# evandez/neuron-descriptions

Measured on AMD Instinct MI355X. Metric: neuron-descriptions/sec (whole node), 4096 neurons x k=15 exemplars, higher is better.
Workload: dtype f32-equivalent: operands split into (hi,lo) f16 pairs (22 significant bits), 3 f16 MFMAs per product, f32 accumulate

## Files before the change

### include/milan_hip.h

```cpp
#ifndef MILAN_HIP_H
#define MILAN_HIP_H

#include <stddef.h>
#include <stdint.h>

#ifdef __cplusplus
extern "C" {
#endif

#if defined(__GNUC__)
#pragma GCC visibility push(default)
#endif

#define MILAN_ABI_VERSION 11

enum {
  MILAN_OK = 0,
  MILAN_ERR_ARG = -1,
  MILAN_ERR_SHAPE = -2,
  MILAN_ERR_STATE = -3,
  MILAN_ERR_WORKSPACE = -4,
  MILAN_ERR_NO_LM = -5
};

// ... 164 lines not shown
                                 milan_stream stream);

size_t milan_exemplar_sort_workspace(int n_units, int64_t n, int pairs);
int milan_exemplar_sketch_compact(const float* src, int64_t src_capacity,
                                  int64_t n, int n_units, int offset, float* dst,
                                  int64_t dst_capacity, int64_t position,
                                  float* extremes, void* workspace,
                                  size_t workspace_bytes, milan_stream stream);

size_t milan_exemplar_sketch_add_workspace(int n_units, int64_t supplied,
                                           const int64_t* capacities,
                                           int n_levels);
int milan_exemplar_sketch_add(const float* hiddens, int batch, int channels, int hw,
                              const int32_t* units, int n_units, int64_t first,
                              int64_t* consumed, float* const* levels,
                              int64_t* firstfree, const int64_t* capacities,
                              int n_levels, const uint8_t* randbits,
                              int64_t n_randbits, int64_t* currentbit,
                              float* extremes, void* workspace,
                              size_t workspace_bytes, milan_stream stream);

int milan_exemplar_rows_extremes(const float* rows, int64_t n_rows, int n_units,
                                 float* extremes, milan_stream stream);

enum { MILAN_SKETCH_COMPACT = 0, MILAN_SKETCH_INSERT = 1, MILAN_SKETCH_MOVE = 2,
       MILAN_SKETCH_HALVE = 3 };
typedef struct milan_sketch_op {
  int32_t kind, src, dst, offset, extremes, reserved;
  int64_t n, position, capacity;
} milan_sketch_op;
int milan_exemplar_sketch_plan_shift(int64_t resolution, int64_t buffersize,
                                     int full_rate, int n_levels,
                                     const int64_t* capacities,
                                     const int64_t* firstfree,
                                     int (*draw_bit)(void*), void* user,
                                     milan_sketch_op* ops, int max_ops, int* n_ops,
                                     int64_t* capacities_out, int64_t* firstfree_out,
                                     int* n_levels_out);

int milan_exemplar_sketch_quantile(const float* const* levels,
                                   const int64_t* firstfree,
                                   const int64_t* capacities, int n_levels,
                                   int n_units, float* extremes, float q,
                                   float* out, void* workspace,
                                   size_t workspace_bytes, milan_stream stream);

int milan_exemplar_render(const float* hiddens, int batch, int channels, int h,
                          int w, const float* images, int img_h, int img_w,
                          const int32_t* cells, int n_cells, const float* levels,
                          const float* mul3, const float* add3, int out_size,
                          int k, uint8_t* out_images, uint8_t* out_masks,
                          uint8_t* out_masked, milan_stream stream);

int milan_conv2d_nhwc(const float* x, int n, int h, int w, int cin,
                      const float* weight_oihw, const float* bias, int cout,
                      int kh, int kw, int stride, int pad, int relu,
                      const float* residual, float* y, int precision,
                      milan_stream stream);

size_t milan_lm_train_workspace_bytes(const milan_ctx* ctx, int rows, int L);
int milan_lm_nll(milan_ctx* ctx, const float* const* params, int n_params,
                 const int64_t* inputs, const int64_t* targets, int rows, int L,
                 float* loss_sum_and_count, void* workspace,
                 size_t workspace_bytes, milan_stream stream);
int milan_lm_train_step(milan_ctx* ctx, const float* const* params,
                        float* const* grads, int n_params,
                        const int64_t* inputs, const int64_t* targets, int rows,
                        int L, float dropout, uint64_t seed,
                        float* loss_sum_and_count, void* workspace,
                        size_t workspace_bytes, milan_stream stream);

size_t milan_lm_grad_workspace_bytes(const milan_ctx* ctx, int rows, int L);
int milan_lm_forward_train(milan_ctx* ctx, const float* const* params,
                           int n_params, const int64_t* inputs, int rows, int L,
                           float dropout, uint64_t seed, float* logprobs_out,
                           float* picked_out, const int64_t* targets,
                           void* workspace, size_t workspace_bytes,
                           milan_stream stream);
int milan_lm_backward(milan_ctx* ctx, const float* const* params,
                      float* const* grads, int n_params, const int64_t* inputs,
                      int rows, int L, float dropout, uint64_t seed,
                      const float* dlogprobs, const float* dpicked,
                      const int64_t* targets, void* workspace,
                      size_t workspace_bytes, milan_stream stream);

size_t milan_decoder_train_workspace_bytes(const milan_ctx* ctx, int rows,
                                           int k, int L);
int milan_decoder_nll(milan_ctx* ctx, const float* const* params, int n_params,
                      const float* features, const int64_t* targets, int rows,
                      int k, int L, float* loss_terms, void* workspace,
                      size_t workspace_bytes, milan_stream stream);
int milan_decoder_train_step(milan_ctx* ctx, const float* const* params,
                             float* const* grads, int n_params,
                             const float* features, const int64_t* targets,
                             int rows, int k, int L, float dropout,
                             uint64_t seed, float regularization_weight,
                             float* loss_terms, void* workspace,
                             size_t workspace_bytes, milan_stream stream);

size_t milan_decoder_grad_workspace_bytes(const milan_ctx* ctx, int rows, int k,
                                          int L);
int milan_decoder_forward_train(milan_ctx* ctx, const float* const* params,
                                int n_params, const float* features,
                                const int64_t* targets, int rows, int k, int L,
                                float dropout, uint64_t seed,
                                float* logprobs_out, float* attentions_out,
// ... 96 lines not shown
```

### neuron-descriptions_amd/csrc/api.hip

```cpp
#include "common.h"

#include <cstdarg>
#include <cstdio>
#include <cstring>

namespace milan {

static thread_local char g_err[1024] = "";

void set_error(const char* fmt, ...) {
  va_list ap;
  va_start(ap, fmt);
  vsnprintf(g_err, sizeof(g_err), fmt, ap);
  va_end(ap);
}

int dev_alloc(milan_ctx* c, void** p, size_t bytes) {
  if (bytes == 0) bytes = 16;
  MILAN_CHECK_HIP(hipMalloc(p, (bytes + 255) & ~size_t(255)));
  c->owned.push_back(*p);
  return 0;
}

__global__ void absmax_kernel(const float* __restrict__ w, long n,
// ... 313 lines not shown
                 int length, int beam_size, int mi, float temperature,
                 int group_size, int64_t* tokens, float* scores,
                 float* predictions, float* attentions, int64_t* beam_tokens,
                 float* beam_scores, int32_t* out_len, void* workspace,
                 size_t workspace_bytes, milan_stream stream) {
  MILAN_REQUIRE(c && features, MILAN_ERR_ARG, "milan_decode: null argument");
  set_status_word(c->status);
  Arena a;
  MILAN_TRY(make_arena(workspace, workspace_bytes, &a));
  DecodeCall d{features, n, k, strategy, length, beam_size, mi, temperature,
               group_size, tokens, scores, predictions, attentions, beam_tokens,
               beam_scores, out_len, workspace, workspace_bytes,
               (hipStream_t)stream, c->precision};
  return decode_maybe_graph(c, d);
}

int milan_set_graph_capture(milan_ctx* c, int enable) {
  MILAN_REQUIRE(c, MILAN_ERR_ARG, "null ctx");
  c->graph_capture = enable != 0;
  if (!enable) {
    for (auto& g : c->graphs)
      if (g.exec) (void)hipGraphExecDestroy(g.exec);
    c->graphs.clear();
  }
  return 0;
}

int milan_graph_stats(const milan_ctx* c, long long* captures, long long* replays) {
  MILAN_REQUIRE(c, MILAN_ERR_ARG, "null ctx");
  if (captures) *captures = c->graph_captures;
  if (replays) *replays = c->graph_replays;
  return 0;
}

int milan_lm_score(milan_ctx* c, const int64_t* seqs, int rows, int L,
                   const int32_t* seq_len, float* out, void* workspace,
                   size_t workspace_bytes, milan_stream stream) {
  MILAN_REQUIRE(c && seqs && out, MILAN_ERR_ARG, "milan_lm_score: null argument");
  set_status_word(c->status);
  Arena a;
  MILAN_TRY(make_arena(workspace, workspace_bytes, &a));
  return decoder_lm_score(c, seqs, rows, L, seq_len, out, a, (hipStream_t)stream);
}

int milan_lm_logprobs(milan_ctx* c, const int64_t* seqs, int rows, int L,
                      float* out, void* workspace, size_t workspace_bytes,
                      milan_stream stream) {
  MILAN_REQUIRE(c && seqs && out, MILAN_ERR_ARG,
                "milan_lm_logprobs: null argument");
  set_status_word(c->status);
  Arena a;
  MILAN_TRY(make_arena(workspace, workspace_bytes, &a));
  return decoder_lm_logprobs(c, seqs, rows, L, out, a, (hipStream_t)stream);
}

int milan_conv2d_nhwc(const float* x, int n, int h, int w, int cin,
                      const float* weight_oihw, const float* bias, int cout,
                      int kh, int kw, int stride, int pad, int relu,
                      const float* residual, float* y, int precision,
                      milan_stream stream) {
  MILAN_REQUIRE(x && weight_oihw && y, MILAN_ERR_ARG, "conv2d: null argument");
  set_status_word(nullptr);
  const bool force_strip = precision == 3, tap_major = precision == 4;
  if (force_strip || tap_major) precision = MILAN_PRECISION_SPLIT_F16;
  MILAN_REQUIRE(!force_strip || MILAN_EXPERIMENTS, MILAN_ERR_ARG,
                "conv2d: the LDS-strip 3x3 kernel is only in an experiments build "
                "(make EXPERIMENTS=1)");
  MILAN_REQUIRE(precision == MILAN_PRECISION_F32 || cin % 32 == 0,
                MILAN_ERR_SHAPE, "conv2d: split-f16 needs cin %% 32 == 0");
  MILAN_REQUIRE(cin % 4 == 0 && n > 0 && cout > 0, MILAN_ERR_SHAPE,
                "conv2d: cin must be a multiple of 4");
  hipStream_t s = (hipStream_t)stream;
  const int K = kh * kw * cin, Kp = (K + 31) / 32 * 32;
  float *wp = nullptr, *zero = nullptr, *xs = nullptr, *wsp = nullptr, *ws3 = nullptr, *wst = nullptr;
  MILAN_CHECK_HIP(hipMalloc((void**)&wp, sizeof(float) * (size_t)cout * Kp));
  MILAN_CHECK_HIP(hipMalloc((void**)&zero, 256));
  MILAN_CHECK_HIP(hipMemsetAsync(zero, 0, 256, s));
  int r = pack_conv_plain(weight_oihw, cout, cin, kh, kw, wp, s);
  if (r == 0) {
    GemmArgs g{};
    const int ho = (h + 2 * pad - kh) / stride + 1, wo = (w + 2 * pad - kw) / stride + 1;
    g.A = x; g.W = wp; g.bias = bias; g.aux = residual; g.C = y;
    g.M = n * ho * wo; g.N = cout; g.K = K; g.Kp = Kp; g.ldc = cout; g.ldaux = cout;
    g.H = h; g.Wd = w; g.Cin = cin; g.Ho = ho; g.Wo = wo; g.KH = kh; g.KW = kw;
    g.stride = stride; g.pad = pad; g.a_pix_stride = cin;
    g.a_img_stride = (long)h * w * cin;
    g.epilogue = residual ? EPI_BIAS_RES_RELU : (relu ? EPI_BIAS_RELU : EPI_BIAS);
    g.zero = zero;
    if (precision == MILAN_PRECISION_SPLIT_F16) {
      const long rows = (long)n * h * w;
      hipError_t e1 = hipMalloc((void**)&xs, sizeof(float) * (size_t)rows * cin);
      hipError_t e2 = hipMalloc((void**)&wsp, sizeof(float) * (size_t)cout * Kp);
      if (e1 != hipSuccess || e2 != hipSuccess) {
        set_error("conv2d: out of memory");
        r = (int)hipErrorOutOfMemory;
      } else {
        r = launch_f32_to_split(x, cin, xs, cin, rows, cin, 1.f, s);
        if (r == 0)
          r = split_weight_into(wp, cout, Kp, wsp, &g.acc_scale,
                                reinterpret_cast<unsigned int*>(zero) + 32, s);
        g.A = xs; g.W = wsp; g.a_split = 1;
        if (r == 0 && !tap_major && kh * kw > 1 && kh * kw <= 32 && K == Kp) {
          if (hipMalloc((void**)&wst, sizeof(float) * (size_t)cout * Kp) == hipSuccess) {
            r = make_slice_major(wsp, cout, kh * kw, cin, 4, 2, wst, s);
            g.Wt = wst;
          }
// ... 155 lines not shown
```

### neuron-descriptions_amd/csrc/common.h

```cpp
#pragma once
#include <hip/hip_runtime.h>
#include <stdint.h>
#include <stddef.h>
#include <string>
#include <vector>
#include <map>

#include "../../include/milan_hip.h"

#ifndef MILAN_EXPERIMENTS
#define MILAN_EXPERIMENTS 0
#endif

namespace milan {

void set_error(const char* fmt, ...);
#define MILAN_CHECK_HIP(expr)                                              \
  do {                                                                     \
    hipError_t _e = (expr);                                                \
    if (_e != hipSuccess) {                                                \
      milan::set_error("%s:%d: %s -> %s", __FILE__, __LINE__, #expr,       \
                       hipGetErrorString(_e));                             \
      return (int)_e;                                                      \
    }                                                                      \
// ... 353 lines not shown
  float *bn1_scale = nullptr, *bn1_shift = nullptr;
  float act_scale = 32.f;
  int act_scale_log2 = 5;
  float *bn1_scale_s = nullptr, *bn1_shift_s = nullptr;
  unsigned* stem_lut = nullptr;
  unsigned* status = nullptr;
  unsigned* calib = nullptr;
  std::vector<milan::Bottleneck> blocks[4];
  float mean[3] = {0.485f, 0.456f, 0.406f}, stdv[3] = {0.229f, 0.224f, 0.225f};
  milan::LinearW init_h, init_c, q2h, k2h, gate, lstm_ih, lstm_hh, out;
  milan::LinearW lstm_cat;
  float *att_w = nullptr, *att_b = nullptr;
  float* embedding = nullptr;
  std::vector<milan::LinearW> lm_ih, lm_hh;
  std::vector<milan::LinearW> lm_cat;
  milan::LinearW lm_out;
  float* lm_embedding = nullptr;
};

namespace milan {
int dev_alloc(milan_ctx* c, void** p, size_t bytes);
int make_split_weight(milan_ctx* c, const float* w, int n, int kp, float** ws,
                      float* ws_inv, hipStream_t s);
int pack_conv_plain(const float* w_oihw, int cout, int cin, int kh, int kw,
                    float* wp, hipStream_t s);
int encoder_finalize(milan_ctx* c, hipStream_t s);
int encoder_rescale(milan_ctx* c, hipStream_t s);
int make_slice_major(const float* ws, int cout, int taps, int cin, int gps, int gb, float* dst,
                     hipStream_t s);
int make_chunk_major(const float* ws, int cout, int cin, float* dst,
                     hipStream_t s);
size_t encoder_workspace(const milan_ctx* c, int n_images, int H, int W);
int encoder_run_spatial(milan_ctx* c, const void* images, int image_dtype,
                        const void* masks, int mask_dtype, int n, int H, int W,
                        float* out, milan::Arena& ws, hipStream_t s);
int encoder_run(milan_ctx* c, const void* images, int image_dtype,
                const void* masks, int mask_dtype, int n_images, int H, int W,
                float* features, Arena& ws, hipStream_t s);
int decoder_finalize(milan_ctx* c, hipStream_t s);
size_t decoder_workspace(const milan_ctx* c, int n, int k, int beam, int length);
int decoder_init_state(milan_ctx* c, const float* features, int n, int k,
                       float* h, float* cc, Arena& ws, hipStream_t s);
int decoder_step(milan_ctx* c, const float* features, int rows, int k,
                 const int64_t* tokens, const float* h, const float* cc,
                 float* h_lm, float* c_lm, float temperature,
                 float* predictions, float* attentions, float* h_out,
                 float* c_out, Arena& ws, hipStream_t s);
int decoder_decode(milan_ctx* c, const float* features, int n, int k,
                   int strategy, int length, int beam, int mi,
                   float temperature, int group_size, int64_t* tokens,
                   float* scores, float* predictions, float* attentions,
                   int64_t* beam_tokens, float* beam_scores, int32_t* out_len,
                   Arena& ws, hipStream_t s);
int decoder_lm_logprobs(milan_ctx* c, const int64_t* seqs, int rows, int L,
                        float* out, milan::Arena& ws, hipStream_t s);
int decoder_lm_score(milan_ctx* c, const int64_t* seqs, int rows, int L,
                     const int32_t* seq_len, float* out, Arena& ws,
                     hipStream_t s);
}
```

### neuron-descriptions_amd/csrc/decoder.hip

```cpp
#include "common.h"
#include <limits>
#include <optional>

namespace milan {

static constexpr float kFloatMin = -3.402823466e+38f;

static const Tensor* find(milan_ctx* c, const std::string& name) {
  auto it = c->raw.find(name);
  return it == c->raw.end() ? nullptr : &it->second;
}

__global__ void pack_rows_kernel(const float* __restrict__ src, int n, int k,
                                 int kp, float* __restrict__ dst) {
  const long total = (long)n * kp;
  for (long idx = blockIdx.x * (long)blockDim.x + threadIdx.x; idx < total;
       idx += (long)gridDim.x * blockDim.x) {
    const int r = idx / kp, col = idx - (long)r * kp;
    dst[idx] = col < k ? src[(long)r * k + col] : 0.f;
  }
}

__device__ inline int lstm_source_row(int i, int hidden) {
  if (!hidden) return i;
// ... 569 lines not shown
  if (lm_logits) {
    const float* y = lm_logits + (long)r * V;
    float my = -INFINITY;
    for (int i = tid; i < V; i += 256) my = fmaxf(my, y[i]);
    my = block_max(my, red);
    float sy = 0.f;
    for (int i = tid; i < V; i += 256) sy += expf(y[i] - my);
    sy = block_sum(sy, red);
    const float lsy = logf(sy);
    for (int i = tid; i < V; i += 256)
      pred[i] = ((pred[i] - mx) - ls) - lambda * ((y[i] - my) - lsy);
  } else {
    for (int i = tid; i < V; i += 256) pred[i] = (pred[i] - mx) - ls;
  }
  if (pred_out) {
    float* po = pred_out + (long)r * pred_stride;
    for (int i = tid; i < V; i += 256) po[i] = pred[i];
  }
  if (k <= 0) return;
  __syncthreads();
  if (last_tok && last_tok[r] == stop) {
    for (int j = tid; j < k; j += 256) {
      cand_v[(long)r * k + j] = j == 0 ? 0.f : kFloatMin;
      cand_i[(long)r * k + j] = j == 0 ? stop : (j - 1 < stop ? j - 1 : j);
    }
    return;
  }
  if (k >= 2 && k <= 256)
    block_topk_fast(pred, V, k, cand_v + (long)r * k, cand_i + (long)r * k,
                    reinterpret_cast<unsigned*>(sm + V + 8));
  else
    block_topk(pred, V, k, cand_v + (long)r * k, cand_i + (long)r * k, red, redi);
}

constexpr int kRowRegs = 24;

__device__ inline float funkey(unsigned key) {
  return __uint_as_float((key & 0x80000000u) ? (key ^ 0x80000000u) : ~key);
}

__global__ __launch_bounds__(256) void row_select_reg_kernel(
    const float* __restrict__ logits, const float* __restrict__ lm_logits,
    float lambda, int V, int k, const int64_t* __restrict__ last_tok, int stop,
    float* __restrict__ cand_v, int* __restrict__ cand_i,
    float* __restrict__ pred_out, long pred_stride, int rank_select) {
  __shared__ float red[8];
  __shared__ unsigned scratch[528];
  const int r = blockIdx.x, tid = threadIdx.x;
  const float* x = logits + (long)r * V;
  float p[kRowRegs];
  float mx = -INFINITY;
#pragma unroll
  for (int j = 0; j < kRowRegs; ++j) {
    const int i = tid + 256 * j;
    p[j] = i < V ? x[i] : -INFINITY;
    mx = fmaxf(mx, p[j]);
  }
  mx = block_max(mx, red);
  float s = 0.f;
#pragma unroll
  for (int j = 0; j < kRowRegs; ++j)
    if (tid + 256 * j < V) s += expf(p[j] - mx);
  s = block_sum(s, red);
  const float ls = logf(s);
  if (lm_logits) {
    const float* y = lm_logits + (long)r * V;
    float q[kRowRegs];
    float my = -INFINITY;
#pragma unroll
    for (int j = 0; j < kRowRegs; ++j) {
      const int i = tid + 256 * j;
      q[j] = i < V ? y[i] : -INFINITY;
      my = fmaxf(my, q[j]);
    }
    my = block_max(my, red);
    float sy = 0.f;
#pragma unroll
    for (int j = 0; j < kRowRegs; ++j)
      if (tid + 256 * j < V) sy += expf(q[j] - my);
    sy = block_sum(sy, red);
    const float lsy = logf(sy);
#pragma unroll
    for (int j = 0; j < kRowRegs; ++j)
      p[j] = ((p[j] - mx) - ls) - lambda * ((q[j] - my) - lsy);
  } else {
#pragma unroll
    for (int j = 0; j < kRowRegs; ++j) p[j] = (p[j] - mx) - ls;
  }
  if (pred_out) {
    float* po = pred_out + (long)r * pred_stride;
#pragma unroll
    for (int j = 0; j < kRowRegs; ++j)
      if (tid + 256 * j < V) po[tid + 256 * j] = p[j];
  }
  if (k <= 0) return;
  float* out_v = cand_v + (long)r * k;
  int* out_i = cand_i + (long)r * k;
  if (last_tok && last_tok[r] == stop) {
    for (int j = tid; j < k; j += 256) {
      out_v[j] = j == 0 ? 0.f : kFloatMin;
      out_i[j] = j == 0 ? stop : (j - 1 < stop ? j - 1 : j);
    }
    return;
  }
  unsigned key[kRowRegs];
#pragma unroll
  for (int j = 0; j < kRowRegs; ++j)
    key[j] = tid + 256 * j < V ? fkey(p[j]) : 0u;
  unsigned* cnt = scratch;
  float* cv = reinterpret_cast<float*>(scratch + 8);
  int* ci = reinterpret_cast<int*>(scratch + 8 + 256);
  if (k >= 2) {
    __shared__ unsigned gk[kGatherCap];
    __shared__ float gp[kGatherCap];
    __shared__ int gi[kGatherCap];
    __shared__ unsigned wave_t[4], gcount;
    unsigned tmax = 0u;
#pragma unroll
    for (int j = 0; j < kRowRegs; ++j) tmax = max(tmax, key[j]);
    const int m_need = (k + 3) >> 2;
    const int lane = tid & 63;
    int rank = 0;
#pragma unroll
    for (int u = 0; u < 64; ++u) {
      const unsigned m = (unsigned)__builtin_amdgcn_readlane((int)tmax, u);
      rank += (m > tmax) || (m == tmax && u < lane);
    }
    if (tid == 0) gcount = 0u;
    if (rank == m_need - 1) wave_t[tid >> 6] = rank_select ? tmax : 0u;
    __syncthreads();
    const unsigned T0 = min(min(wave_t[0], wave_t[1]), min(wave_t[2], wave_t[3]));
    if (T0 != 0u) {
#pragma unroll
      for (int j = 0; j < kRowRegs; ++j)
        if (key[j] >= T0) {
          const unsigned q = atomicAdd(&gcount, 1u);
          if (q < (unsigned)kGatherCap) { gk[q] = key[j]; gp[q] = p[j]; gi[q] = tid + 256 * j; }
        }
      __syncthreads();
      const int total = (int)gcount;
      if (total <= kGatherCap) {
        for (int c0 = tid; c0 < total; c0 += 256) {
          const unsigned mk = gk[c0];
          const int mi = gi[c0];
          int r2 = 0;
          for (int u = 0; u < total; ++u) {
            const unsigned ok = gk[u];
            r2 += (ok > mk) || (ok == mk && gi[u] < mi);
          }
          if (r2 < k) { out_v[r2] = gp[c0]; out_i[r2] = mi; }
        }
        return;
      }
    }
    __syncthreads();
  }
  unsigned kmax = 0u, kmin = 0xFFFFFFFFu;
#pragma unroll
  for (int j = 0; j < kRowRegs; ++j)
    if (tid + 256 * j < V) { kmax = max(kmax, key[j]); kmin = min(kmin, key[j]); }
  for (int o = 32; o > 0; o >>= 1) {
    kmax = max(kmax, (unsigned)__shfl_xor((int)kmax, o));
    kmin = min(kmin, (unsigned)__shfl_xor((int)kmin, o));
  }
  __syncthreads();
  if ((tid & 63) == 0) { cnt[tid >> 6] = kmax; cnt[4 + (tid >> 6)] = kmin; }
  __syncthreads();
  unsigned hi = max(max(cnt[0], cnt[1]), max(cnt[2], cnt[3]));
  unsigned lo = min(min(cnt[4], cnt[5]), min(cnt[6], cnt[7]));
  if (k == 1) {
    int best = 0x7fffffff;
#pragma unroll
    for (int j = 0; j < kRowRegs; ++j)
      if (key[j] == hi && tid + 256 * j < V) best = min(best, tid + 256 * j);
    for (int o = 32; o > 0; o >>= 1) best = min(best, __shfl_xor(best, o));
    __syncthreads();
    if ((tid & 63) == 0) cnt[tid >> 6] = (unsigned)best;
    __syncthreads();
    if (tid == 0) {
      out_i[0] = (int)min(min(cnt[0], cnt[1]), min(cnt[2], cnt[3]));
      out_v[0] = funkey(hi);
    }
    return;
  }
  for (int it = 0; it < 32 && lo < hi; ++it) {
    const unsigned mid = lo + ((hi - lo) >> 1) + ((hi - lo) & 1u);
    int c = 0;
#pragma unroll
    for (int j = 0; j < kRowRegs; ++j) c += key[j] >= mid;
    for (int o = 32; o > 0; o >>= 1) c += __shfl_xor(c, o);
    __syncthreads();
    if ((tid & 63) == 0) cnt[tid >> 6] = (unsigned)c;
    __syncthreads();
    const int total = (int)(cnt[0] + cnt[1] + cnt[2] + cnt[3]);
    if (total >= k) lo = mid; else hi = mid - 1u;
  }
  const unsigned T = lo;
  __syncthreads();
  if (tid == 0) { cnt[4] = 0u; cnt[5] = 0u; }
  __syncthreads();
#pragma unroll
  for (int j = 0; j < kRowRegs; ++j) {
    const int i = tid + 256 * j;
// ... 531 lines not shown
    launch_context(b->att, features, rows, rpn, k, F, b->ctx, s);
    {
      GemmArgs g = split_lin(c->gate, xs + E, ldx, EPI_BIAS_SIGMUL, b->ctx, F);
      g.out_split = 1;
      MILAN_TRY(launch_gemm(g, s));
    }
    hipLaunchKernelGGL(embed_split_kernel, dim3(nblk((long)rows * (E / 8))),
                       dim3(256), 0, s, c->embedding, tok, rows, E, xs, ldx);
    {
      const LinearW& w = c->lstm_cat;
      const bool cell = w.gate_interleaved;
      GemmArgs g = cell ? linear_args(xs, ldx, w.ws, w.b, hn, H, rows, w.n, w.k,
                                      EPI_LSTM, c->zero, cc, H)
                        : linear_args(xs, ldx, w.ws, w.b, b->gates, 4 * H, rows,
                                      w.n, w.k, EPI_BIAS, c->zero);
      if (cell) { g.C2 = cn; g.Cs = hs2; }
      g.a_split = 1;
      g.acc_scale = w.ws_inv;
      g.Cin = ldx;
      g.A2 = hs; g.K1 = ldx; g.H2 = 1; g.W2d = 1; g.stride2 = 1;
      g.a2_pix_stride = H; g.a2_img_stride = H;
      MILAN_TRY(launch_gemm(g, s));
      if (!cell) {
        hipLaunchKernelGGL(lstm_pointwise_kernel, dim3(nblk((long)rows * H)),
                           dim3(256), 0, s, b->gates, cc, rows, H, hn, cn);
        hs2 = hs;
        MILAN_TRY(launch_f32_to_split(hn, H, hs2, H, rows, H, 1.f, s));
      }
    }
    hs = hs2;
    MILAN_TRY(launch_gemm(split_lin(c->out, b->logits, V, EPI_BIAS, nullptr, 0), s));
    MILAN_CHECK_HIP(hipGetLastError());
    return 0;
  }
  MILAN_TRY(lin(c, h, H, c->q2h, b->q, A, rows, EPI_BIAS, s));
  launch_attend(b->q, keys, c->att_w, c->att_b, rows, rpn, k, A, b->att, s);
  launch_context(b->att, features, rows, rpn, k, F, b->ctx, s);
  MILAN_TRY(lin(c, h, H, c->gate, b->x + E, ldx, rows, EPI_BIAS_SIGMUL, s, b->ctx, F));
  hipLaunchKernelGGL(embed_kernel, dim3(nblk((long)rows * E)), dim3(256), 0, s,
                     c->embedding, tok, rows, E, b->x, ldx);
  MILAN_TRY(lstm_layer(c, b->x, ldx, c->lstm_ih, h, H, c->lstm_hh, c->lstm_cat,
                       b->gates, cc, hn, cn, rows, s));
  MILAN_TRY(lin(c, hn, H, c->out, b->logits, V, rows, EPI_BIAS, s));
  MILAN_CHECK_HIP(hipGetLastError());
  return 0;
}

static size_t row_select_lds(int V) { return sizeof(float) * (V + 8 + 528); }

static int launch_row_select(const float* logits, const float* lm_logits,
                             float lambda, int rows, int V, int k,
                             const int64_t* last_tok, int stop, float* cand_v,
                             int* cand_i, float* pred_out, long pred_stride,
                             hipStream_t s) {
  if (V <= kRowRegs * 256 && k <= 256 && (k <= 1 || k <= V)) {
    static const int rank_select = [] {
      const char* e = getenv("MILAN_ROW_SELECT");
      return (e && e[0] == 't') ? 0 : 1;
    }();
    hipLaunchKernelGGL(row_select_reg_kernel, dim3(rows), dim3(256), 0, s,
                       logits, lm_logits, lambda, V, k, last_tok, stop, cand_v,
                       cand_i, pred_out, pred_stride, rank_select);
    MILAN_CHECK_HIP(hipGetLastError());
    return 0;
  }
  const size_t lds = row_select_lds(V);
  MILAN_REQUIRE(lds <= 160 * 1024, MILAN_ERR_SHAPE,
                "vocab_size %d too large for the row-select kernel", V);
  if (lds > 64 * 1024)
    MILAN_TRY(ensure_lds_attr(reinterpret_cast<const void*>(row_select_kernel), (int)lds));
  hipLaunchKernelGGL(row_select_kernel, dim3(rows), dim3(256), lds, s, logits,
                     lm_logits, lambda, V, k, last_tok, stop, cand_v, cand_i,
                     pred_out, pred_stride);
  MILAN_CHECK_HIP(hipGetLastError());
  return 0;
}

int decoder_step(milan_ctx* c, const float* features, int rows, int k,
                 const int64_t* tokens, const float* h, const float* cc,
                 float* h_lm, float* c_lm, float temperature, float* predictions,
                 float* attentions, float* h_out, float* c_out, Arena& ws,
                 hipStream_t s) {
  MILAN_TRY(check_dims(c, k));
  const bool mi = h_lm != nullptr;
  MILAN_REQUIRE((h_lm == nullptr) == (c_lm == nullptr), MILAN_ERR_ARG,
                "state must have both h_lm and c_lm or neither");
  MILAN_REQUIRE(!mi || c->d.has_lm, MILAN_ERR_NO_LM,
                "state has h_lm or c_lm, but decoder has no lm");
  DecBuf b;
  dec_plan(c, rows, k, 1, 1, mi, ws, &b);
  c->scratch = ws.off <= ws.size ? b.scratch : nullptr;
  c->scratch_floats = b.scratch_floats;
  MILAN_REQUIRE(ws.off <= ws.size, MILAN_ERR_WORKSPACE,
                "step: workspace too small (%zu needed)", ws.off);
  MILAN_TRY(project_keys(c, features, rows * k, b.keys, s));
  MILAN_TRY(step_core(c, features, b.keys, rows, 1, k, tokens, h, cc, h_out,
                      c_out, &b, s));
  const float* lm_logits = nullptr;
  if (mi) {
    LmState st{h_lm, c_lm, rows};
    MILAN_TRY(lm_step(c, tokens, rows, st, b.lm[0], b.lm_emb, b.lm_gates,
                      b.lm_logits, s));
    const size_t bytes = sizeof(float) * (size_t)rows * c->d.lm_hidden_size *
                         c->d.lm_layers;
    MILAN_CHECK_HIP(hipMemcpyAsync(h_lm, b.lm[0].h, bytes, hipMemcpyDeviceToDevice, s));
    MILAN_CHECK_HIP(hipMemcpyAsync(c_lm, b.lm[0].c, bytes, hipMemcpyDeviceToDevice, s));
    lm_logits = b.lm_logits;
  }
  MILAN_TRY(launch_row_select(b.logits, lm_logits, temperature, rows,
                              c->d.vocab_size, 0, nullptr, 0, nullptr, nullptr,
                              predictions, c->d.vocab_size, s));
  if (attentions)
    MILAN_CHECK_HIP(hipMemcpyAsync(attentions, b.att,
                                   sizeof(float) * (size_t)rows * k,
                                   hipMemcpyDeviceToDevice, s));
  return 0;
}

__global__ void gather_col_kernel(const int64_t* __restrict__ seqs, long rows,
                                  long lds, int t, int64_t* __restrict__ out) {
  const long r = blockIdx.x * (long)blockDim.x + threadIdx.x;
  if (r < rows) out[r] = seqs[r * lds + t];
}

static bool lm_split_ok(const milan_ctx* c, int rows) {
  const milan_dims& d = c->d;
  if (c->precision != MILAN_PRECISION_SPLIT_F16 || !c->scratch || !c->lm_out.ws ||
      d.lm_layers < 1 || d.lm_layers > 2 || d.lm_embedding_size % 16 ||
// ... 523 lines not shown
```

### neuron-descriptions_amd/milan_amd/hip.py

```python
import ctypes
import os
import pathlib
import weakref
from typing import Dict, Optional, Sequence

import torch

LIB_PATH = pathlib.Path(os.environ.get('MILAN_LIB') or
                       pathlib.Path(__file__).resolve().parent / 'lib' / 'libmilan_hip.so')
EXP_LIB_PATH = pathlib.Path(__file__).resolve().parent / 'lib' / 'libmilan_hip_exp.so'

GREEDY, FORCED, BEAM, RERANK = 0, 1, 2, 3
PRECISION_F32, PRECISION_SPLIT_F16, PRECISION_F16 = 0, 1, 2
PRECISIONS = {'f32': PRECISION_F32, 'split_f16': PRECISION_SPLIT_F16, 'f16': PRECISION_F16}
FUSE_CHAIN, FUSE_CHAIN_WIDE, FUSE_STEM, FUSE_CONV3, FUSE_SKIP_EMPTY, FUSE_BNECK, FUSE_SPARSE_TAIL = 1, 2, 4, 8, 16, 32, 64
SKETCH_COMPACT, SKETCH_INSERT, SKETCH_MOVE, SKETCH_HALVE = 0, 1, 2, 3
STATUS_SATURATED, STATUS_NONFINITE_INPUT = 1, 2
KERNEL_FAMILIES = ('other', 'pp32_256', 'pp32_128', 'split_other', 'f32', 'chain',
                   'chain_wide', 'stem', 'conv3', 'f16', 'pp32t_256', 'bneck')


class SketchOp(ctypes.Structure):
    _fields_ = [('kind', ctypes.c_int32), ('src', ctypes.c_int32),
                ('dst', ctypes.c_int32), ('offset', ctypes.c_int32),
# ... 135 lines not shown
    'milan_lm_train_workspace_bytes': (_SZ, [_P, _I, _I]),
    'milan_lm_nll': (_I, [_P, _P, _I, _P, _P, _I, _I, _P, _P, _SZ, _P]),
    'milan_lm_train_step':
        (_I, [_P, _P, _P, _I, _P, _P, _I, _I, _F, ctypes.c_uint64, _P, _P,
              _SZ, _P]),
    'milan_lm_grad_workspace_bytes': (_SZ, [_P, _I, _I]),
    'milan_lm_forward_train':
        (_I, [_P, _P, _I, _P, _I, _I, _F, ctypes.c_uint64, _P, _P, _P, _P, _SZ,
              _P]),
    'milan_lm_backward':
        (_I, [_P, _P, _P, _I, _P, _I, _I, _F, ctypes.c_uint64, _P, _P, _P, _P,
              _SZ, _P]),
    'milan_decoder_train_workspace_bytes': (_SZ, [_P, _I, _I, _I]),
    'milan_decoder_nll':
        (_I, [_P, _P, _I, _P, _P, _I, _I, _I, _P, _P, _SZ, _P]),
    'milan_decoder_train_step':
        (_I, [_P, _P, _P, _I, _P, _P, _I, _I, _I, _F, ctypes.c_uint64, _F, _P,
              _P, _SZ, _P]),
    'milan_decoder_grad_workspace_bytes': (_SZ, [_P, _I, _I, _I]),
    'milan_decoder_forward_train':
        (_I, [_P, _P, _I, _P, _P, _I, _I, _I, _F, ctypes.c_uint64, _P, _P, _P,
              _SZ, _P]),
    'milan_decoder_backward':
        (_I, [_P, _P, _P, _I, _P, _P, _I, _I, _I, _F, ctypes.c_uint64, _P, _P,
              _P, _P, _SZ, _P]),
    'milan_clip_create': (_I, [ctypes.POINTER(_P), _I,
                               ctypes.POINTER(ClipDims)]),
    'milan_clip_destroy': (None, [_P]),
    'milan_clip_set_weight':
        (_I, [_P, ctypes.c_char_p, _P,
              ctypes.POINTER(ctypes.c_int64), _I]),
    'milan_clip_finalize_weights': (_I, [_P, _P]),
    'milan_clip_image_workspace_bytes': (_SZ, [_P, _I, _I]),
    'milan_clip_encode_images':
        (_I, [_P, _P, _I, _I, _P, ctypes.c_uint64, _I,
              ctypes.POINTER(_F), _P, _P, _SZ, _P]),
    'milan_clip_text_workspace_bytes': (_SZ, [_P, _I, _I]),
    'milan_clip_encode_texts': (_I, [_P, _P, _I, _I, _P, _P, _SZ, _P]),
    'milan_clip_rerank_scores':
        (_I, [_P, _P, _P, _P, _I, _I, _I, _I, _I, _F, _P, _P]),
    'milan_bert_create': (_I, [ctypes.POINTER(_P), _I,
                               ctypes.POINTER(BertDims)]),
    'milan_bert_destroy': (None, [_P]),
    'milan_bert_set_weight':
        (_I, [_P, ctypes.c_char_p, _P,
              ctypes.POINTER(ctypes.c_int64), _I]),
    'milan_bert_finalize_weights': (_I, [_P, _P]),
    'milan_bert_encode_workspace_bytes': (_SZ, [_P, _I, _I]),
    'milan_bert_encode': (_I, [_P, _P, _P, _I, _I, _I, _I, _P, _P, _SZ, _P]),
    'milan_bert_score_pairs': (_I, [_P, _P, _P, _P, _P, _I, _I, _I, _P, _P]),
    'milan_conv2d_nhwc':
        (_I, [_P, _I, _I, _I, _I, _P, _P, _I, _I, _I, _I, _I, _I, _P, _P, _I,
              _P]),
}

PROBED = ('milan_lm_grad_workspace_bytes', 'milan_lm_forward_train',
          'milan_lm_backward')

_lib = None


def load_library(path: Optional[os.PathLike] = None) -> ctypes.CDLL:
    global _lib
    if _lib is not None and path is None:
        return _lib
    p = pathlib.Path(path) if path is not None else LIB_PATH
    if not p.exists():
        raise HipUnavailableError(
            f'{p} not found: build it with `python -c "import __graft_entry__ '
            'as g; g.build()"` (or `make -C neuron-descriptions_amd/csrc`). '
            'There is no CPU fallback for the MILAN hot path.')
    try:
        lib = ctypes.CDLL(str(p))
    except OSError as error:
        raise HipUnavailableError(f'cannot load {p}: {error}') from error
    for name, (restype, argtypes) in SIGNATURES.items():
        if name in PROBED and not hasattr(lib, name):
            continue
        fn = getattr(lib, name)
        fn.restype = restype
        fn.argtypes = argtypes
    if lib.milan_abi_version() != ABI_VERSION:
        raise HipUnavailableError(
            f'{p} has C-ABI version {lib.milan_abi_version()}, this binding '
            f'needs {ABI_VERSION} (struct milan_dims differs): rebuild it')
    if path is None:
        _lib = lib
    return lib


def require_device(device: torch.device) -> torch.device:
    device = torch.device(device)
    if device.type != 'cuda' or not torch.cuda.is_available():
        raise HipUnavailableError(
            'milan_amd computes only on an AMD GPU (torch device "cuda" under '
            f'ROCm); got device={device}, cuda.is_available()='
            f'{torch.cuda.is_available()}. There is no CPU fallback.')
    if device.index is None:
        device = torch.device('cuda', torch.cuda.current_device())
    return device


def _check(code: int) -> None:
    if code == 0:
        return
    msg = load_library().milan_last_error().decode(errors='replace')
    if code in (ERR_ARG, ERR_SHAPE, ERR_NO_LM):
        raise ValueError(msg)
    raise RuntimeError(f'libmilan_hip error {code}: {msg}')


def _ptr(t: Optional[torch.Tensor]) -> Optional[int]:
    return None if t is None else t.data_ptr()


def _stream(device: torch.device) -> int:
    return torch.cuda.current_stream(device).cuda_stream


def _dev(t: torch.Tensor, device: torch.device, dtype=None) -> torch.Tensor:
    if dtype is not None and t.dtype != dtype:
        t = t.to(dtype)
    if t.device != device:
        t = t.to(device)
    return t.contiguous()


_LIVE_CONTEXTS: 'weakref.WeakSet' = weakref.WeakSet()


# ... 1053 lines not shown

    def score_pairs(self, emb: torch.Tensor, offsets: torch.Tensor,
                    weights: torch.Tensor, cand: torch.Tensor,
                    ref: torch.Tensor) -> torch.Tensor:
        emb = _dev(emb, self.device, torch.float32)
        offsets = _dev(offsets, self.device, torch.int32)
        weights = _dev(weights, self.device, torch.float32)
        cand = _dev(cand, self.device, torch.int32)
        ref = _dev(ref, self.device, torch.int32)
        if (weights.numel() != emb.shape[0] or cand.numel() != ref.numel() or
                emb.shape[1] != self.dims.width):
            raise ValueError('score_pairs: emb / weights / cand / ref disagree')
        pairs = cand.numel()
        out = torch.empty((pairs, 3), device=self.device)
        with torch.cuda.device(self.device):
            _check(self.lib.milan_bert_score_pairs(
                emb.data_ptr(), offsets.data_ptr(), weights.data_ptr(),
                cand.data_ptr(), ref.data_ptr(), pairs, offsets.numel() - 1,
                emb.shape[1], out.data_ptr(), _stream(self.device)))
        return out


def profile_enable(enable: bool) -> None:
    _check(load_library().milan_profile_enable(int(enable)))


def profile_read():
    ms, fl, n = ctypes.c_double(), ctypes.c_double(), ctypes.c_longlong()
    _check(load_library().milan_profile_read(ctypes.byref(ms), ctypes.byref(fl),
                                             ctypes.byref(n)))
    return ms.value, fl.value, n.value


STAGES = ('other', 'enc_input', 'enc_stem', 'enc_stem_tail', 'enc_layer1',
          'enc_layer2', 'enc_layer3', 'enc_layer4', 'enc_pool', 'dec_init',
          'dec_search', 'dec_lm')


def profile_read_stages() -> Dict[str, Dict[str, float]]:
    table = (ctypes.c_double * (len(STAGES) * 6))()
    _check(load_library().milan_profile_read_stages(table))
    keys = ('region_ms', 'regions', 'gemm_ms', 'gemm_flops', 'gemm_launches',
            'gemm_bytes')
    return {name: dict(zip(keys, table[i * 6:i * 6 + 6]))
            for i, name in enumerate(STAGES)}


def profile_read_kernels() -> Dict[str, Dict[str, float]]:
    table = (ctypes.c_double * (len(KERNEL_FAMILIES) * 4))()
    _check(load_library().milan_profile_read_kernels(table))
    keys = ('ms', 'flops', 'launches', 'bytes')
    return {name: dict(zip(keys, table[i * 4:i * 4 + 4]))
            for i, name in enumerate(KERNEL_FAMILIES)}


def conv2d_nhwc(x: torch.Tensor,
                weight: torch.Tensor,
                bias: Optional[torch.Tensor] = None,
                stride: int = 1,
                padding: int = 0,
                relu: bool = False,
                residual: Optional[torch.Tensor] = None,
                precision: str = 'f32',
                lib: Optional[ctypes.CDLL] = None) -> torch.Tensor:
    lib = lib if lib is not None else load_library()
    device = require_device(x.device)
    n, h, w, cin = x.shape
    cout, cin_w, kh, kw = weight.shape
    assert cin_w == cin
    ho = (h + 2 * padding - kh) // stride + 1
    wo = (w + 2 * padding - kw) // stride + 1
    y = torch.empty(n, ho, wo, cout, device=device)
    x, weight = x.contiguous(), weight.contiguous()
    with torch.cuda.device(device):
        _check(
            lib.milan_conv2d_nhwc(x.data_ptr(), n, h, w, cin,
                                  weight.data_ptr(), _ptr(bias), cout, kh, kw,
                                  stride, padding, int(relu), _ptr(residual),
                                  y.data_ptr(), _CONV_PRECISIONS[precision],
                                  _stream(device)))
    return y


def make_dims(state_dict: Dict[str, torch.Tensor],
              n_vocab_tokens: int,
              blocks: Sequence[int] = (3, 4, 23, 3)) -> Dims:
    d = Dims()
    sd = state_dict
    pre = 'encoder.encoder.model.'
    width = kind = None
    if pre + 'features.0.weight' in sd:
        kind, width = TRUNK_ALEXNET, sd[pre + 'features.0.weight'].shape[0]
    elif pre + 'conv1.weight' in sd:
        width = sd[pre + 'conv1.weight'].shape[0]
        kind = (TRUNK_BOTTLENECK if pre + 'layer1.0.conv3.weight' in sd else
                TRUNK_BASIC)
    if 'lstm.weight_hh' in sd:
        hidden = sd['lstm.weight_hh'].shape[1]
        emb = sd['embedding.weight'].shape[1]
        feat = sd['lstm.weight_ih'].shape[1] - emb
        att = sd['attend.query_to_hidden.weight'].shape[0]
        vocab = sd['output.1.weight'].shape[0]
    else:
        hidden, emb, att, vocab = 4, 4, 4, n_vocab_tokens + 4
        feat = _FEATURE_MULT[kind] * width if kind is not None else 4
    if width is None:
# ... 26 lines not shown
```

Before: 1312.

## Rework register row-select top-k with ballot radix threshold and packed key ranking

In the register-resident row-select kernel, the per-wave threshold is now found by a 32-step ballot radix search instead of 64 readlane comparisons. Candidates are gathered with one atomic per wave plus mbcnt offsets rather than one atomic per element, and key and index are packed into one 64-bit word. Ranking is split across the four waves, which write partial counts to LDS, replacing the per-thread O(total) rank loop. Loads are clamped so they stay unconditional. The change also exposes a milan_row_select API and Python hook for testing, at the cost of extra LDS and an added barrier.

```diff
diff --git a/include/milan_hip.h b/include/milan_hip.h
--- a/include/milan_hip.h
+++ b/include/milan_hip.h
@@ -240,6 +240,11 @@
                           int k, uint8_t* out_images, uint8_t* out_masks,
                           uint8_t* out_masked, milan_stream stream);
 
+int milan_row_select(const float* logits, const float* lm_logits, float lambda,
+                     int rows, int vocab, int k, const int64_t* last_tok, int stop,
+                     float* cand_v, int* cand_i, float* pred_out, int variant,
+                     milan_stream stream);
+
 int milan_conv2d_nhwc(const float* x, int n, int h, int w, int cin,
                       const float* weight_oihw, const float* bias, int cout,
                       int kh, int kw, int stride, int pad, int relu,
diff --git a/neuron-descriptions_amd/csrc/api.hip b/neuron-descriptions_amd/csrc/api.hip
--- a/neuron-descriptions_amd/csrc/api.hip
+++ b/neuron-descriptions_amd/csrc/api.hip
@@ -389,6 +389,17 @@
   Arena a;
   MILAN_TRY(make_arena(workspace, workspace_bytes, &a));
   return decoder_lm_logprobs(c, seqs, rows, L, out, a, (hipStream_t)stream);
+}
+
+int milan_row_select(const float* logits, const float* lm_logits, float lambda,
+                     int rows, int vocab, int k, const int64_t* last_tok, int stop,
+                     float* cand_v, int* cand_i, float* pred_out, int variant,
+                     milan_stream stream) {
+  MILAN_REQUIRE(logits && (k == 0 || (cand_v && cand_i)), MILAN_ERR_ARG,
+                "milan_row_select: null argument");
+  return decoder_row_select(logits, lm_logits, lambda, rows, vocab, k, last_tok,
+                            stop, cand_v, cand_i, pred_out, variant,
+                            (hipStream_t)stream);
 }
 
 int milan_conv2d_nhwc(const float* x, int n, int h, int w, int cin,
diff --git a/neuron-descriptions_amd/csrc/common.h b/neuron-descriptions_amd/csrc/common.h
--- a/neuron-descriptions_amd/csrc/common.h
+++ b/neuron-descriptions_amd/csrc/common.h
@@ -429,6 +429,10 @@
                    float* scores, float* predictions, float* attentions,
                    int64_t* beam_tokens, float* beam_scores, int32_t* out_len,
                    Arena& ws, hipStream_t s);
+int decoder_row_select(const float* logits, const float* lm_logits, float lambda,
+                       int rows, int V, int k, const int64_t* last_tok, int stop,
+                       float* cand_v, int* cand_i, float* pred_out, int variant,
+                       hipStream_t s);
 int decoder_lm_logprobs(milan_ctx* c, const int64_t* seqs, int rows, int L,
                         float* out, milan::Arena& ws, hipStream_t s);
 int decoder_lm_score(milan_ctx* c, const int64_t* seqs, int rows, int L,
diff --git a/neuron-descriptions_amd/csrc/decoder.hip b/neuron-descriptions_amd/csrc/decoder.hip
--- a/neuron-descriptions_amd/csrc/decoder.hip
+++ b/neuron-descriptions_amd/csrc/decoder.hip
@@ -645,15 +645,19 @@
   float mx = -INFINITY;
 #pragma unroll
   for (int j = 0; j < kRowRegs; ++j) {
-    const int i = tid + 256 * j;
-    p[j] = i < V ? x[i] : -INFINITY;
+    const float v = x[min((unsigned)(tid + 256 * j), (unsigned)(V - 1))];
+    p[j] = tid < V - 256 * j ? v : -INFINITY;
     mx = fmaxf(mx, p[j]);
   }
   mx = block_max(mx, red);
   float s = 0.f;
 #pragma unroll
-  for (int j = 0; j < kRowRegs; ++j)
-    if (tid + 256 * j < V) s += expf(p[j] - mx);
+  for (int g = 0; g < kRowRegs; g += 4)
+    if (256 * g < V) {
+#pragma unroll
+      for (int j = g; j < g + 4; ++j)
+        if (tid < V - 256 * j) s += expf(p[j] - mx);
+    }
   s = block_sum(s, red);
   const float ls = logf(s);
   if (lm_logits) {
@@ -662,15 +666,19 @@
     float my = -INFINITY;
 #pragma unroll
     for (int j = 0; j < kRowRegs; ++j) {
-      const int i = tid + 256 * j;
-      q[j] = i < V ? y[i] : -INFINITY;
+      const float v = y[min((unsigned)(tid + 256 * j), (unsigned)(V - 1))];
+      q[j] = tid < V - 256 * j ? v : -INFINITY;
       my = fmaxf(my, q[j]);
     }
     my = block_max(my, red);
     float sy = 0.f;
 #pragma unroll
-    for (int j = 0; j < kRowRegs; ++j)
-      if (tid + 256 * j < V) sy += expf(q[j] - my);
+    for (int g = 0; g < kRowRegs; g += 4)
+      if (256 * g < V) {
+#pragma unroll
+        for (int j = g; j < g + 4; ++j)
+          if (tid < V - 256 * j) sy += expf(q[j] - my);
+      }
     sy = block_sum(sy, red);
     const float lsy = logf(sy);
 #pragma unroll
@@ -684,7 +692,7 @@
     float* po = pred_out + (long)r * pred_stride;
 #pragma unroll
     for (int j = 0; j < kRowRegs; ++j)
-      if (tid + 256 * j < V) po[tid + 256 * j] = p[j];
+      if (tid < V - 256 * j) po[tid + 256 * j] = p[j];
   }
   if (k <= 0) return;
   float* out_v = cand_v + (long)r * k;
@@ -699,49 +707,79 @@
   unsigned key[kRowRegs];
 #pragma unroll
   for (int j = 0; j < kRowRegs; ++j)
-    key[j] = tid + 256 * j < V ? fkey(p[j]) : 0u;
+    key[j] = tid < V - 256 * j ? fkey(p[j]) : 0u;
   unsigned* cnt = scratch;
   float* cv = reinterpret_cast<float*>(scratch + 8);
   int* ci = reinterpret_cast<int*>(scratch + 8 + 256);
   if (k >= 2) {
-    __shared__ unsigned gk[kGatherCap];
-    __shared__ float gp[kGatherCap];
-    __shared__ int gi[kGatherCap];
+    __shared__ __attribute__((aligned(16))) unsigned long long gc[kGatherCap];
+    __shared__ __attribute__((aligned(16))) unsigned part[kGatherCap * 4];
     __shared__ unsigned wave_t[4], gcount;
     unsigned tmax = 0u;
 #pragma unroll
     for (int j = 0; j < kRowRegs; ++j) tmax = max(tmax, key[j]);
     const int m_need = (k + 3) >> 2;
     const int lane = tid & 63;
-    int rank = 0;
-#pragma unroll
-    for (int u = 0; u < 64; ++u) {
-      const unsigned m = (unsigned)__builtin_amdgcn_readlane((int)tmax, u);
-      rank += (m > tmax) || (m == tmax && u < lane);
+    const int wave = __builtin_amdgcn_readfirstlane(tid >> 6);
+    unsigned sel = 0u;
+#pragma unroll
+    for (int b = 31; b >= 0; --b) {
+      const unsigned cand = sel | (1u << b);
+      if (__popcll(__ballot(tmax >= cand)) >= m_need) sel = cand;
     }
     if (tid == 0) gcount = 0u;
-    if (rank == m_need - 1) wave_t[tid >> 6] = rank_select ? tmax : 0u;
+    if (lane == 0) wave_t[wave] = rank_select ? sel : 0u;
     __syncthreads();
     const unsigned T0 = min(min(wave_t[0], wave_t[1]), min(wave_t[2], wave_t[3]));
     if (T0 != 0u) {
+      unsigned long long mask[kRowRegs];
+      int wc = 0;
+#pragma unroll
+      for (int j = 0; j < kRowRegs; ++j) {
+        mask[j] = __ballot(key[j] >= T0);
+        wc += __popcll(mask[j]);
+      }
+      unsigned base = 0u;
+      if (lane == 0) base = atomicAdd(&gcount, (unsigned)wc);
+      base = (unsigned)__builtin_amdgcn_readfirstlane((int)base);
 #pragma unroll
       for (int j = 0; j < kRowRegs; ++j)
-        if (key[j] >= T0) {
-          const unsigned q = atomicAdd(&gcount, 1u);
-          if (q < (unsigned)kGatherCap) { gk[q] = key[j]; gp[q] = p[j]; gi[q] = tid + 256 * j; }
+        if (mask[j] != 0ull) {
+          const unsigned q = __builtin_amdgcn_mbcnt_hi(
+              (unsigned)(mask[j] >> 32), __builtin_amdgcn_mbcnt_lo((unsigned)mask[j], base));
+          if (key[j] >= T0 && q < (unsigned)kGatherCap)
+            gc[q] = ((unsigned long long)key[j] << 32) | (unsigned)~(tid + 256 * j);
+          base += (unsigned)__popcll(mask[j]);
         }
       __syncthreads();
       const int total = (int)gcount;
       if (total <= kGatherCap) {
+        const int quarter = (total + 3) >> 2;
+        const int u0 = wave * quarter;
+        const int u1 = min(u0 + quarter, total);
+        for (int cb = 0; cb < total; cb += 128) {
+          const int ca = cb + lane, cc = ca + 64;
+          const unsigned long long ma = ca < total ? gc[ca] : ~0ull;
+          const unsigned long long mc = cc < total ? gc[cc] : ~0ull;
+          int ra = 0, rc = 0;
+#pragma unroll 4
+          for (int u = u0; u < u1; ++u) {
+            const unsigned long long o = gc[u];
+            ra += o > ma;
+            rc += o > mc;
+          }
+          if (ca < total) part[ca * 4 + wave] = (unsigned)ra;
+          if (cc < total) part[cc * 4 + wave] = (unsigned)rc;
+        }
+        __syncthreads();
         for (int c0 = tid; c0 < total; c0 += 256) {
-          const unsigned mk = gk[c0];
-          const int mi = gi[c0];
-          int r2 = 0;
-          for (int u = 0; u < total; ++u) {
-            const unsigned ok = gk[u];
-            r2 += (ok > mk) || (ok == mk && gi[u] < mi);
+          const uint4 pr = *reinterpret_cast<const uint4*>(&part[c0 * 4]);
+          const int r2 = (int)((pr.x + pr.y) + (pr.z + pr.w));
+          if (r2 < k) {
+            const unsigned long long m = gc[c0];
+            out_v[r2] = funkey((unsigned)(m >> 32));
+            out_i[r2] = (int)~(unsigned)m;
           }
-          if (r2 < k) { out_v[r2] = gp[c0]; out_i[r2] = mi; }
         }
         return;
       }
@@ -1379,8 +1417,8 @@
                              float lambda, int rows, int V, int k,
                              const int64_t* last_tok, int stop, float* cand_v,
                              int* cand_i, float* pred_out, long pred_stride,
-                             hipStream_t s) {
-  if (V <= kRowRegs * 256 && k <= 256 && (k <= 1 || k <= V)) {
+                             hipStream_t s, bool force_lds = false) {
+  if (!force_lds && V <= kRowRegs * 256 && k <= 256 && (k <= 1 || k <= V)) {
     static const int rank_select = [] {
       const char* e = getenv("MILAN_ROW_SELECT");
       return (e && e[0] == 't') ? 0 : 1;
@@ -1401,6 +1439,19 @@
                      pred_out, pred_stride);
   MILAN_CHECK_HIP(hipGetLastError());
   return 0;
+}
+
+int decoder_row_select(const float* logits, const float* lm_logits, float lambda,
+                       int rows, int V, int k, const int64_t* last_tok, int stop,
+                       float* cand_v, int* cand_i, float* pred_out, int variant,
+                       hipStream_t s) {
+  MILAN_REQUIRE(rows > 0 && V > 0 && k >= 0 && k <= V, MILAN_ERR_SHAPE,
+                "row_select: need rows > 0 and 0 <= k <= V (rows %d, V %d, k %d)",
+                rows, V, k);
+  MILAN_REQUIRE(variant == 0 || variant == 1, MILAN_ERR_ARG,
+                "row_select: variant is 0 (as the decoder picks) or 1 (LDS kernel)");
+  return launch_row_select(logits, lm_logits, lambda, rows, V, k, last_tok, stop,
+                           cand_v, cand_i, pred_out, V, s, variant == 1);
 }
 
 int decoder_step(milan_ctx* c, const float* features, int rows, int k,
diff --git a/neuron-descriptions_amd/milan_amd/hip.py b/neuron-descriptions_amd/milan_amd/hip.py
--- a/neuron-descriptions_amd/milan_amd/hip.py
+++ b/neuron-descriptions_amd/milan_amd/hip.py
@@ -211,10 +211,13 @@
     'milan_conv2d_nhwc':
         (_I, [_P, _I, _I, _I, _I, _P, _P, _I, _I, _I, _I, _I, _I, _P, _P, _I,
               _P]),
+    'milan_row_select':
+        (_I, [_P, _P, ctypes.c_float, _I, _I, _I, _P, _I, _P, _P, _P, _I, _P]),
 }
 
 PROBED = ('milan_lm_grad_workspace_bytes', 'milan_lm_forward_train',
           'milan_lm_backward')
+PROBED_HOOKS = ('milan_row_select',)
 
 _lib = None
 
@@ -234,7 +237,7 @@
     except OSError as error:
         raise HipUnavailableError(f'cannot load {p}: {error}') from error
     for name, (restype, argtypes) in SIGNATURES.items():
-        if name in PROBED and not hasattr(lib, name):
+        if name in PROBED + PROBED_HOOKS and not hasattr(lib, name):
             continue
         fn = getattr(lib, name)
         fn.restype = restype
@@ -1394,6 +1397,42 @@
     keys = ('ms', 'flops', 'launches', 'bytes')
     return {name: dict(zip(keys, table[i * 4:i * 4 + 4]))
             for i, name in enumerate(KERNEL_FAMILIES)}
+
+
+def row_select(logits: torch.Tensor,
+               k: int,
+               lm_logits: Optional[torch.Tensor] = None,
+               temperature: float = 0.0,
+               last_tok: Optional[torch.Tensor] = None,
+               stop: int = 0,
+               variant: int = 0,
+               want_pred: bool = True,
+               lib: Optional[ctypes.CDLL] = None):
+    lib = lib if lib is not None else load_library()
+    if not hasattr(lib, 'milan_row_select'):
+        raise HipUnavailableError(
+            'the loaded libmilan_hip has no milan_row_select: rebuild it (or '
+            'unset MILAN_LIB)')
+    device = require_device(logits.device)
+    rows, vocab = logits.shape
+    logits = logits.contiguous().float()
+    if lm_logits is not None:
+        assert lm_logits.shape == logits.shape
+        lm_logits = lm_logits.contiguous().float()
+    if last_tok is not None:
+        assert last_tok.shape == (rows,) and last_tok.dtype == torch.int64
+        last_tok = last_tok.contiguous()
+    vals = torch.empty(rows, k, device=device)
+    idx = torch.empty(rows, k, dtype=torch.int32, device=device)
+    pred = torch.empty(rows, vocab, device=device) if want_pred else None
+    with torch.cuda.device(device):
+        _check(
+            lib.milan_row_select(logits.data_ptr(), _ptr(lm_logits),
+                                 float(temperature), rows, vocab, k,
+                                 _ptr(last_tok), stop, vals.data_ptr(),
+                                 idx.data_ptr(), _ptr(pred), variant,
+                                 _stream(device)))
+    return vals, idx, pred
 
 
 def conv2d_nhwc(x: torch.Tensor,
```

Measured after the change: 1321, median of 4. About the same (+0.6%).
